# KatiaJDL/CenterPoly

Hardware: AMD Instinct MI355X
Metric: inference img/s @2048x1024 DLA-34 (1 GPU) (higher is better)
Workload: dtype f32 I/O; split-bf16 x3 contraction (a*b ~ ah*bh + ah*bl + al*bh on bf16 MFMA, ~2^-16 per product) in the convolutions, the heads and DCNv2; f32 accumulate; 1 GPU; BASELINE config 2: DLA-34 + DCNv2, 1x3x1024x2048 synthetic, 16-vertex cartesian head, K=128, forward + sigmoid + NMS/top-k/decode; parallelism=single

## Files before the change

### centerpoly_amd/_C.py

```python
import ctypes
import os
from ctypes import POINTER, Structure, c_char_p, c_float, c_int32, c_int64, c_size_t, c_void_p

import torch

_HERE = os.path.dirname(os.path.abspath(__file__))
LIB_PATH = os.path.join(_HERE, "csrc", "libcenterpoly_hip.so")

CP_OK = 0
REP = {"cartesian": 0, "polar": 1, "polar_fixed": 2}
HEATMAP_UMICH, HEATMAP_ELLIPSE = 0, 1
L1_PLAIN, L1_POLAR, L1_POLAR_FIXED, L1_RELU20, L1_SMOOTH = 0, 1, 2, 3, 4
DCN_BWD_EXACT_F32, DCN_BWD_NARROW_TILES = 1, 2
DCN_CONTRACTION = {"f32": 0, "bf16x3": 1, "bf16x3_region": 3}


class DcnShape(Structure):
    _fields_ = [(n, c_int32) for n in ("B", "Cin", "H", "W", "Cout", "kh", "kw", "stride", "pad",
                                       "dil", "deformable_groups")]


class TargetShape(Structure):
    _fields_ = [(n, c_int32) for n in ("B", "max_objs", "nbr_points", "num_classes", "out_h", "out_w",
                                       "rep", "no_reorder_flip")]
# ... 54 lines not shown
    "cp_color_aug_normalize": (c_int32, [_P, c_int64, c_int32, _P, _P, _P, _P, _P, _P, c_size_t, _P]),
    "cp_sample_inputs_workspace_bytes": (c_size_t, [c_int32] * 3),
    "cp_sample_inputs_batch": (c_int32, [_P] * 7 + [c_int32] * 3 + [_P, _P, c_size_t, _P]),
    "cp_instance_masks": (c_int32, [_P, _P, c_int32, c_int32, c_int32, c_int32, _P, _P, _P]),
    "cp_writer_instances": (c_int32, [_P, c_int32, c_int32, c_float, _P, c_int32, _P, _P, _P, _P, _P, _P, _P]),
    "cp_class_instance_masks": (c_int32, [_P, _P, _P, c_int32, c_int32, c_int32, c_int32, _P, _P, _P]),
    "cp_class_writer_instances": (c_int32, [_P, c_int32, c_int32, c_float, c_int32, _P, c_int32] + [_P] * 9),
    "cp_annot_id_instances_workspace_bytes": (c_size_t, []),
    "cp_annot_id_instances": (c_int32, [_P, c_int32, c_int32, _P, c_int32, c_int32, c_int32, _P, _P, _P, _P, _P,
                                        c_size_t, _P]),
    "cp_polygon_masks_workspace_bytes": (c_size_t, [c_int32, c_int32]),
    "cp_polygon_masks": (c_int32, [_P, _P, c_int32, c_int32, c_int32, _P, _P, _P, c_size_t, _P]),
    "cp_annot_rays_ids": (c_int32, [_P, c_int32, c_int32, _P, _P, c_int32, c_int32, _P, _P]),
    "cp_annot_rays_masks": (c_int32, [_P, c_int32, c_int32, _P, c_int32, c_int32, _P, _P]),
    "cp_polygon_paint_workspace_bytes": (c_size_t, [c_int32, c_int32]),
    "cp_polygon_paint": (c_int32, [_P, _P, _P, c_int32, c_int32, c_int32, c_int32, _P, _P, c_size_t, _P]),
    "cp_render_overlay_workspace_bytes": (c_size_t, [c_int32, c_int32]),
    "cp_render_overlay": (c_int32, [_P, c_int32, c_int32, _P, c_int32, c_int32, _P, _P, _P, _P, c_int32, _P, c_int32, _P,
                                    c_int32, _P, _P, _P, c_size_t, _P]),
    "cp_render_heatmap": (c_int32, [_P, c_int32, c_int32, c_int32, c_int32, _P, _P, _P, _P, c_int32, c_int32, _P, _P]),
    "cp_oracle_map": (c_int32, [_P, _P] + [c_int32] * 5 + [_P, _P]),
    "cp_id_histogram": (c_int32, [_P, c_int32, c_int32, _P, _P]),
    "cp_instance_overlaps_workspace_bytes": (c_size_t, [c_int32] * 4),
    "cp_instance_overlaps": (c_int32, [_P, c_int32, _P, c_int32, c_int32, _P, c_int32, _P, c_int32, _P, _P, _P, _P,
                                       c_size_t, _P]),
    "cp_polydet_post_process": (c_int32, [_P, _P, c_float, c_int32, c_int32, c_int32, _P, _P]),
    "cp_polydet_targets_workspace_bytes": (c_size_t, [POINTER(TargetShape)]),
    "cp_polydet_targets": (c_int32, [POINTER(TargetShape)] + [_P] * 19 + [_P, c_size_t, _P]),
    "cp_polydet_targets_ex": (c_int32, [POINTER(TargetShape), c_int32] + [_P] * 19 + [_P, c_size_t, _P]),
    "cp_polydet_dense_targets": (c_int32, [POINTER(TargetShape), _P, _P, c_size_t, _P, _P, _P]),
    "cp_conv_direct_supported": (c_int32, [c_int32] * 5),
    "cp_conv_direct_wgrad_supported": (c_int32, [c_int32] * 5),
    "cp_conv_direct_wgrad": (c_int32, [_P, _P, _P] + [c_int32] * 8 + [_P]),
    "cp_conv_direct_forward": (c_int32, [_P, _P, _P, _P] + [c_int32] * 9 + [_P]),
    "cp_conv_direct_forward_ex": (c_int32, [_P, _P, _P, _P] + [c_int32] * 10 + [_P]),
    "cp_conv3x3_mfma_supported": (c_int32, [c_int32] * 4),
    "cp_conv3x3_mfma_weight_bytes": (c_size_t, [c_int32] * 2),
    "cp_conv3x3_mfma_prepare": (c_int32, [_P, c_int32, c_int32, c_int32, _P, _P]),
    "cp_conv3x3_mfma_forward": (c_int32, [_P, _P, _P, _P, _P] + [c_int32] * 6 + [_P]),
    "cp_conv_mfma_weight_bytes": (c_size_t, [c_int32] * 3),
    "cp_conv_mfma_prepare": (c_int32, [_P, c_int32, c_int32, c_int32, c_int32, _P, _P]),
    "cp_conv3x3_s2_wgrad_supported": (c_int32, [c_int32] * 4),
    "cp_conv3x3_s2_wgrad": (c_int32, [_P, _P, _P] + [c_int32] * 5 + [_P]),
    "cp_conv7x7_c3_supported": (c_int32, [c_int32] * 4),
    "cp_conv7x7_c3_weight_bytes": (c_size_t, [c_int32]),
    "cp_conv7x7_c3_prepare": (c_int32, [_P, c_int32, _P, _P]),
    "cp_conv7x7_c3_forward": (c_int32, [_P, _P, _P, _P] + [c_int32] * 6 + [_P]),
    "cp_conv_mfma_prepare_blocks": (c_int32, [c_int32] * 3),
    "cp_conv_mfma_prepare_batch": (c_int32, [_P, c_int32, c_int32, _P]),
    "cp_conv_mfma_forward": (c_int32, [_P, _P, c_int32, _P, _P, _P, _P] + [c_int32] * 6 + [_P]),
    "cp_conv_mfma_forward_strided": (c_int32, [_P, _P, c_int32, _P, _P, _P, _P] + [c_int32] * 7 + [_P]),
    "cp_dla_base_pair_supported": (c_int32, [c_int32] * 2),
    "cp_dla_base_pair_forward": (c_int32, [_P] * 6 + [c_int32] * 3 + [_P]),
    "cp_conv_mfma_forward_split": (c_int32, [_P, c_int32, _P, _P, _P, _P] + [c_int32] * 9 + [_P]),
    "cp_activation_split": (c_int32, [_P, _P] + [c_int32] * 4 + [_P]),
    "cp_activation_unsplit": (c_int32, [_P, _P] + [c_int32] * 4 + [_P]),
    "cp_conv1x1_stream_supported": (c_int32, [_P, c_int32, c_int32, c_int32, c_int32]),
    "cp_conv1x1_stream_weight_bytes": (c_size_t, [c_int32] * 2),
    "cp_conv1x1_stream_prepare": (c_int32, [_P, c_int32, c_int32, _P, _P]),
    "cp_conv1x1_stream_forward": (c_int32, [_P, _P, c_int32, _P, _P, _P, _P] + [c_int32] * 5 + [_P]),
    "cp_conv1x1_stream_form": (c_int32, [c_int32] * 5),
    "cp_conv1x1_stream_forward_form": (c_int32, [_P, _P, c_int32, _P, _P, _P, _P] + [c_int32] * 7 + [_P]),
    "cp_conv3x3_stream_supported": (c_int32, [c_int32] * 4),
    "cp_conv3x3_stream_form": (c_int32, [c_int32] * 5),
    "cp_conv3x3_stream_forward": (c_int32, [_P] * 5 + [c_int32] * 6 + [_P]),
    "cp_conv3x3_stream_forward_form": (c_int32, [_P] * 5 + [c_int32] * 8 + [_P]),
    "cp_conv_mfma_input_grad_relu_workspace_bytes": (c_size_t, [c_int32] * 4),
    "cp_conv_mfma_input_grad_relu": (c_int32, [_P] * 5 + [c_int32] * 6 + [_P, c_size_t, _P]),
    "cp_conv3x3_s2_input_grad": (c_int32, [_P, _P, _P, _P] + [c_int32] * 5 + [_P]),
    "cp_conv3x3_mfma_wgrad_supported": (c_int32, [c_int32] * 4),
    "cp_conv3x3_mfma_wgrad": (c_int32, [_P, _P, _P] + [c_int32] * 5 + [_P]),
    "cp_conv_mfma_wgrad": (c_int32, [_P, _P, _P] + [c_int32] * 6 + [_P]),
    "cp_heads_fused_w2_bytes": (c_size_t, [c_int32]),
    "cp_heads_fused_prepare_w2": (c_int32, [_P, c_int32, c_int32, _P, _P]),
    "cp_heads_fused_forward": (c_int32, [_P, _P, _P, _P, _P, _P, _P] + [c_int32] * 6 + [_P]),
    "cp_maxpool2x2_forward": (c_int32, [_P, _P] + [c_int32] * 4 + [_P]),
    "cp_maxpool2x2_backward": (c_int32, [_P, _P, _P] + [c_int32] * 4 + [_P]),
    "cp_conv1x1_act_forward": (c_int32, [_P, c_int64, _P, c_int32, _P, _P, _P, c_int32, c_int32, c_int32, c_int64, _P]),
    "cp_soft_nms": (c_int32, [_P, c_int32, c_int32, c_float, c_float, c_float, c_int32]),
    "cp_soft_nms_device": (c_int32, [_P, c_int32, _P, _P, c_int32, c_float, c_float, c_float, c_int32, _P, _P]),
    "cp_merge_detections_workspace_bytes": (c_size_t, [c_int32] * 4),
    "cp_merge_detections": (c_int32, [_P] + [c_int32] * 6 + [c_float] * 3 + [c_int32, _P, _P, _P, c_size_t, _P]),
    "cp_polydet_decode_workspace_bytes": (c_size_t, [c_int32] * 5),
    "cp_polydet_decode": (c_int32, [_P, _P, _P, _P] + [c_int32] * 7 + [_P, _P, _P, _P, c_size_t, _P]),
    "cp_polydet_decode_ex": (c_int32, [_P, _P, _P, _P] + [c_int32] * 8 + [_P, _P, _P, _P, c_size_t, _P]),
    "cp_sigmoid_focal_workspace_bytes": (c_size_t, [c_int64]),
    "cp_sigmoid_focal_forward": (c_int32, [_P, _P, c_int64, _P, _P, _P, c_size_t, _P]),
    "cp_sigmoid_focal_backward": (c_int32, [_P, _P, c_int64, _P, _P, _P, _P]),
    "cp_gather_l1_forward": (c_int32, [_P, _P, _P, _P, _P] + [c_int32] * 6 + [c_float, _P, _P]),
    "cp_gather_l1_backward": (c_int32, [_P, _P, _P, _P, _P] + [c_int32] * 6 + [c_float, _P, _P, _P]),
    "cp_mse_workspace_bytes": (c_size_t, []),
    "cp_mse_forward": (c_int32, [_P, _P, c_int64, _P, _P, c_size_t, _P]),
    "cp_mse_backward": (c_int32, [_P, _P, c_int64, _P, _P, _P]),
    "cp_dense_l1_workspace_bytes": (c_size_t, []),
    "cp_dense_l1_forward": (c_int32, [_P, _P, _P, c_int64, c_float, _P, _P, c_size_t, _P]),
    "cp_dense_l1_backward": (c_int32, [_P, _P, _P, c_int64, _P, _P, _P, _P]),
    "cp_poly_iou_order_workspace_bytes": (c_size_t, [c_int32] * 3),
    "cp_poly_iou_order_forward": (c_int32, [_P, _P, _P, _P] + [c_int32] * 6 + [_P, _P, _P, _P,
                                                                               c_size_t, _P]),
    "cp_poly_iou_order_backward": (c_int32, [_P, _P, _P, _P] + [c_int32] * 6 + [_P, _P, _P, _P,
                                                                                c_size_t, _P]),
}

EXPORTS = tuple(_SIGNATURES)


# ... 52 lines not shown

    def release(self):
        self.block, self.off, self.key = None, 0, None

    def take(self, shape, device):
        n = 1
        for d in shape:
            n *= int(d)
        nbytes = (n * 4 + 255) // 256 * 256
        if nbytes > self.BLOCK // 8 or n == 0:
            return torch.zeros(tuple(shape), dtype=torch.float32, device=device)
        dev = torch.device(device)
        if dev.type == "cuda" and dev.index is None:
            dev = torch.device("cuda", torch.cuda.current_device())
        key = (dev, torch.cuda.current_stream(dev).cuda_stream)
        if self.block is None or self.key != key or self.off + nbytes > self.BLOCK:
            self.block = torch.zeros(self.BLOCK // 4, dtype=torch.float32, device=device)
            self.off, self.key = 0, key
        t = self.block[self.off // 4: self.off // 4 + n].view(tuple(shape))
        self.off += nbytes
        return t


_zero_pool = _ZeroPool()


def zeros(shape, device):
    return _zero_pool.take(shape, device)


def release_zero_pool():
    _zero_pool.release()


class _NoEvent(object):
    def record(self):
        pass


class KernelTimer(object):

    def __init__(self, watch=None):
        self.records = {}
        self.watch = watch

    def start(self, key):
        if self.watch is not None and key not in self.watch:
            return _NoEvent()
        ev = (torch.cuda.Event(enable_timing=True), torch.cuda.Event(enable_timing=True))
        self.records.setdefault(key, []).append(ev)
        ev[0].record()
        return ev[1]

    def summary(self):
        torch.cuda.synchronize()
        out = {}
        for key, evs in self.records.items():
            ms = [a.elapsed_time(b) for a, b in evs]
            out[key] = {"launches": len(ms), "avg_ms": sum(ms) / len(ms), "min_ms": min(ms)}
        return out


kernel_timer = None
```

### centerpoly_amd/models/networks/conv3x3.py

```python

import weakref

import torch
import torch.nn.functional as F

from ... import _C
from .prepared import prepared

_ENABLED = True
_WGRAD = True
MIN_CIN = 24
MIN_WORKGROUPS = 128
STREAM_1X1 = "auto"
STREAM_3X3 = "auto"


def _workgroups(B, cout, H, W):
    return B * ((W + 31) // 32) * ((H + 3) // 4) * ((cout + 31) // 32)


def _fills(B, cin, cout, H, W):
    n = _workgroups(B, cout, H, W)
    return n >= MIN_WORKGROUPS or (cin >= 256 and n >= 16)

# ... 231 lines not shown
    return out


def block_infer(x, conv1, wb1, conv2, wb2, skip):
    planes = wb1[0].shape[0]
    if not (_ENABLED and x.is_cuda and planes % 32 == 0 and tuple(wb1[0].shape[2:]) == (3, 3)
            and tuple(wb2[0].shape[2:]) == (3, 3) and conv2.stride == (1, 1)):
        return None
    B, _, H, W = x.shape
    s = conv1.stride[0]
    Ho, Wo = (H - 1) // s + 1, (W - 1) // s + 1
    if planes < MIN_CIN or not _fills(B, planes, planes, Ho, Wo) \
            or not _C.lib().cp_conv3x3_mfma_supported(planes, planes, Ho, Wo) or (skip is not None and not skip.is_contiguous()):
        return None
    y = conv_infer([x], conv1, wb1[0], wb1[1], None, True, conv=conv1, out_split=True)
    if y is None:
        return None
    z = conv_infer([y], conv2, wb2[0], wb2[1], skip, True, conv=conv2, x_split=True)
    if z is None:
        raise _C.NativeError("block_infer: the second convolution refused a split tensor its first convolution wrote")
    return z


def s2_input_grad(xshape, weight, go):
    L = _C.lib()
    B, cin, H, W = xshape
    cout = weight.shape[0]
    Ho, Wo = (H - 1) // 2 + 1, (W - 1) // 2 + 1
    if not (_ENABLED and go.is_cuda and go.dtype == torch.float32 and tuple(weight.shape[2:]) == (3, 3)
            and tuple(go.shape) == (B, cout, Ho, Wo) and cout >= MIN_CIN and L.cp_conv3x3_mfma_supported(cout, cin, Ho, Wo)
            and cin * H * W * 4 < 0x7FFFFFF0 and _fills(B, cout, cin, Ho, Wo)):
        return None
    go = go.contiguous()
    gx = torch.empty(xshape, dtype=torch.float32, device=go.device)
    end = _C.kernel_timer.start(("conv3x3s2_igrad", cout, cin, Ho, Wo, B)) if _C.kernel_timer is not None else None
    wp = _prepare(weight, cout, cin, 6)
    _C.check(L.cp_conv3x3_s2_input_grad(_C.ptr(go), _C.ptr(wp), None, _C.ptr(gx), B, cin, H, W, cout, _C.stream()),
             "cp_conv3x3_s2_input_grad")
    if end is not None:
        end.record()
    return gx


def stem_infer(x, conv, w, bias, relu):
    if not (_ENABLED and x.is_cuda and x.dtype == torch.float32 and x.dim() == 4 and conv.kernel_size == (7, 7)
            and conv.stride in ((1, 1), (2, 2)) and conv.padding == (3, 3) and conv.dilation == (1, 1) and conv.groups == 1
            and conv.in_channels == 3 and x.shape[1] == 3 and conv.padding_mode == "zeros"):
        return None
    L = _C.lib()
    B, _, H, W = x.shape
    cout, stride = w.shape[0], conv.stride[0]
    if not L.cp_conv7x7_c3_supported(cout, H, W, stride) or B > 65535:
        return None

    def build():
        wp = torch.empty(L.cp_conv7x7_c3_weight_bytes(cout), dtype=torch.uint8, device=w.device)
        _C.check(L.cp_conv7x7_c3_prepare(_C.ptr(w.contiguous()), cout, _C.ptr(wp), _C.stream()), "cp_conv7x7_c3_prepare")
        return wp
    wp, _ = prepared(conv, "stem", (w,), build)
    out = torch.empty((B, cout, (H - 1) // stride + 1, (W - 1) // stride + 1), dtype=torch.float32, device=x.device)
    _C.check(L.cp_conv7x7_c3_forward(_C.ptr(x.contiguous()), _C.ptr(wp), _C.ptr(bias), _C.ptr(out), B, H, W, cout,
                                     stride, 1 if relu else 0, _C.stream()), "cp_conv7x7_c3_forward")
    return out


def s2_weight_grad(x, weight, go):
    L = _C.lib()
    B, cin, H, W = x.shape
    cout = weight.shape[0]
    if not (_ENABLED and _WGRAD and x.is_cuda and x.dtype == torch.float32 and tuple(weight.shape[2:]) == (3, 3)
            and cin >= MIN_CIN and L.cp_conv3x3_s2_wgrad_supported(cin, cout, H, W)
            and tuple(go.shape) == (B, cout, (H - 1) // 2 + 1, W // 2)):
        return None
    gw = _C.zeros(weight.shape, weight.device)
    end = _C.kernel_timer.start(("conv3x3s2_wgrad", cin, cout, H, W, B)) if _C.kernel_timer is not None else None
    _C.check(L.cp_conv3x3_s2_wgrad(_C.ptr(x), _C.ptr(go.contiguous()), _C.ptr(gw), B, cin, H, W, cout, _C.stream()),
             "cp_conv3x3_s2_wgrad")
    if end is not None:
        end.record()
    return gw


class _Conv3x3Fn(torch.autograd.Function):

    @staticmethod
    def forward(ctx, x, weight, stride=1):
        ctx.save_for_backward(x, weight)
        ctx.stride = stride
        cout, cin = weight.shape[0], weight.shape[1]
        return _launch(x, _prepare(weight, cin, cout, False), None, None, cout, False, weight.shape[2] * weight.shape[3],
                       stride)

    @staticmethod
    def backward(ctx, go):
        x, weight = ctx.saved_tensors
        go = go.contiguous()
        if ctx.stride != 1:
            gx = None
            if ctx.needs_input_grad[0]:
                gx = s2_input_grad(x.shape, weight, go)
                if gx is None:
                    gx = torch.nn.grad.conv2d_input(x.shape, weight, go, stride=ctx.stride, padding=1)
            gw = None
            if ctx.needs_input_grad[1]:
                gw = s2_weight_grad(x, weight, go)
                if gw is None:
                    gw = torch.nn.grad.conv2d_weight(x, weight.shape, go, stride=ctx.stride, padding=1)
            return gx, gw, None
        return grads(x, weight, go, ctx.needs_input_grad[0], ctx.needs_input_grad[1], min_k=MIN_CIN) + (None,)


class _Conv3x3SkipFn(torch.autograd.Function):

    @staticmethod
    def forward(ctx, x, weight):
        ctx.save_for_backward(x, weight)
# ... 234 lines not shown
```

### centerpoly_amd/models/networks/pose_dla_dcn.py

```python
import math
import os

import numpy as np
import torch
import torch.nn.functional as F
from torch import nn

from ... import _C
from .DCNv2.dcn_v2 import DCN, conv_bias
from . import conv3x3
from .conv3x3 import conv_infer, conv_raw
from .prepared import prepared, release_inference

HEADS_FUSED = True
CONV_DIRECT_WGRAD = True

BN_MOMENTUM = 0.1


def _bn(c):
    return nn.BatchNorm2d(c, momentum=BN_MOMENTUM)



# ... 57 lines not shown
        gx = gw = None
        if weight.shape[2] == 3 and stride == 1 and pad == 1 and conv3x3.mfma_enabled():
            gx, gw = conv3x3.grads(x, weight, go, ctx.needs_input_grad[0], ctx.needs_input_grad[1] and not direct_w)
        elif ctx.needs_input_grad[0]:
            if weight.shape[2] == 3 and stride == 2 and pad == 1 and conv3x3.mfma_enabled():
                gx = conv3x3.s2_input_grad(tuple(x.shape), weight, go)
            if gx is None:
                gx = torch.nn.grad.conv2d_input(x.shape, weight, go, stride=stride, padding=pad)
        if ctx.needs_input_grad[1] and gw is None:
            L = _C.lib()
            B, cin, H, W = x.shape
            cout, k = weight.shape[0], weight.shape[2]
            if direct_w and L.cp_conv_direct_wgrad_supported(cin, cout, k, stride, pad):
                gw = _C.zeros(weight.shape, weight.device)
                rc = L.cp_conv_direct_wgrad(_C.ptr(x), _C.ptr(go), _C.ptr(gw), B, cin, H, W, cout, k, stride, pad,
                                            _C.stream())
                if rc == -2:
                    gw = None
                else:
                    _C.check(rc, "cp_conv_direct_wgrad")
            if gw is None:
                gw = torch.nn.grad.conv2d_weight(x, weight.shape, go, stride=stride, padding=pad)
        return gx, gw, None, None


def conv_train(conv, x):
    kh, kw = conv.kernel_size
    if (x.is_cuda and x.dtype == torch.float32 and conv.bias is None and kh == kw and conv.groups == 1
            and conv.dilation == (1, 1) and conv.stride[0] == conv.stride[1] and conv.padding[0] == conv.padding[1]
            and x.shape[1] * x.shape[2] * x.shape[3] * 4 < 0x70000000
            and _C.lib().cp_conv_direct_supported(conv.in_channels, conv.out_channels, kh, conv.stride[0],
                                                  conv.padding[0])):
        return _DirectConvFn.apply(x.contiguous(), conv.weight, conv.stride[0], conv.padding[0])
    if conv.bias is None:
        return conv_raw(conv, x)
    return conv(x)


def _base_pair(dla, x):
    c0, c1 = dla.level0[0], dla.level1[0]
    if not (x.is_cuda and x.dtype == torch.float32 and x.dim() == 4 and conv3x3.mfma_enabled()
            and (c0.in_channels, c0.out_channels, c0.kernel_size, c0.stride, c0.padding, c0.dilation, c0.groups)
            == (16, 16, (3, 3), (1, 1), (1, 1), (1, 1), 1)
            and (c1.in_channels, c1.out_channels, c1.kernel_size, c1.stride, c1.padding, c1.dilation, c1.groups)
            == (16, 32, (3, 3), (2, 2), (1, 1), (1, 1), 1)):
        return None
    B, _, H, W = x.shape
    L = _C.lib()
    if not L.cp_dla_base_pair_supported(H, W) or B > 65535:
        return None
    (w0, b0), (w1, b1) = dla._folded[1], dla._folded[2]
    x = x.contiguous()
    out = torch.empty((B, 32, (H - 1) // 2 + 1, (W - 1) // 2 + 1), dtype=torch.float32, device=x.device)
    end = _C.kernel_timer.start(("conv_base_pair", 16, 32, H, W, B)) if _C.kernel_timer is not None else None
    rc = L.cp_dla_base_pair_forward(_C.ptr(x), _C.ptr(w0.contiguous()), _C.ptr(b0), _C.ptr(w1.contiguous()), _C.ptr(b1),
                                    _C.ptr(out), B, H, W, _C.stream())
    if rc == -2:
        return None
    _C.check(rc, "cp_dla_base_pair_forward")
    if end is not None:
        end.record()
    return out


def _conv_folded(x, conv, wb, relu=False, residual=None):
    if residual is None:
        y = None
        if conv.kernel_size == (7, 7) and x.is_cuda:
            y = conv3x3.stem_infer(x, conv, wb[0], wb[1], relu)
        if y is None:
            y = _conv_direct(x, conv, wb, relu)
        if y is not None:
            return y
    if x.is_cuda:
        y = conv_infer([x], conv, wb[0], wb[1], residual, relu, conv=conv)
        if y is not None:
            return y
    if not x.is_cuda:
        y = F.conv2d(x, wb[0], wb[1], conv.stride, conv.padding, conv.dilation, conv.groups)
        if residual is not None:
            y = y + residual
        return F.relu_(y) if relu else y
    y = F.conv2d(x, wb[0], None, conv.stride, conv.padding, conv.dilation, conv.groups)
    B, C, H, W = y.shape
    if not y.is_contiguous() or (H * W) % 4 != 0 or (residual is not None and not residual.is_contiguous()):
        y = y + wb[1].view(1, -1, 1, 1)
        if residual is not None:
            y = y + residual
        return F.relu_(y) if relu else y
    rc = _C.lib().cp_bias_act_inplace(_C.ptr(y), _C.ptr(wb[1]), _C.ptr(residual), B, C, H * W,
                                      1 if relu else 0, _C.stream())
    _C.check(rc, "cp_bias_act_inplace")
    return y


class _MaxPool2x2Fn(torch.autograd.Function):

    @staticmethod
    def forward(ctx, x):
        B, C, H, W = x.shape
        out = torch.empty((B, C, H // 2, W // 2), dtype=torch.float32, device=x.device)
        _C.check(_C.lib().cp_maxpool2x2_forward(_C.ptr(x), _C.ptr(out), B, C, H, W, _C.stream()), "cp_maxpool2x2_forward")
        ctx.save_for_backward(x)
        return out

    @staticmethod
    def backward(ctx, go):
        (x,) = ctx.saved_tensors
        B, C, H, W = x.shape
        gx = torch.empty_like(x)
        _C.check(_C.lib().cp_maxpool2x2_backward(_C.ptr(x), _C.ptr(go.contiguous()), _C.ptr(gx), B, C, H, W,
                                                 _C.stream()), "cp_maxpool2x2_backward")
# ... 222 lines not shown
                    if bottom.is_cuda:
                        bn_act(self.project[1], conv_train(self.project[0], bottom), relu=False)
                    else:
                        self.project(bottom)
        elif _use_folded(self):
            residual = _conv_folded(bottom, self.project[0], self._folded)
        else:
            residual = bn_act(self.project[1], conv_train(self.project[0], bottom), relu=False)
        if self.level_root:
            children.append(bottom)
        if Tree.share_pool and self.levels > 1 and not torch.is_grad_enabled() and self._same_pool(self.tree1):
            x1 = self.tree1(x, residual, bottom=bottom)
        else:
            x1 = self.tree1(x, residual)
        if self.levels == 1:
            return self.root(self.tree2(x1), x1, *children)
        children.append(x1)
        return self.tree2(x1, children=children)


class DLA(nn.Module):
    def __init__(self, levels, channels, num_classes=1000, block=BasicBlock, residual_root=False,
                 linear_root=False):
        super().__init__()
        self.channels, self.num_classes = channels, num_classes
        c = channels
        self.base_layer = nn.Sequential(nn.Conv2d(3, c[0], 7, 1, 3, bias=False), _bn(c[0]),
                                        nn.ReLU(inplace=True))
        self.level0 = self._conv_level(c[0], c[0], levels[0])
        self.level1 = self._conv_level(c[0], c[1], levels[1], stride=2)
        for i in range(2, 6):
            setattr(self, "level%d" % i, Tree(levels[i], block, c[i - 1], c[i], 2,
                                              level_root=i > 2, root_residual=residual_root))

    @staticmethod
    def _conv_level(inplanes, planes, convs, stride=1, dilation=1):
        mods = []
        for i in range(convs):
            mods += [nn.Conv2d(inplanes, planes, 3, stride if i == 0 else 1, dilation, dilation,
                               bias=False), _bn(planes), nn.ReLU(inplace=True)]
            inplanes = planes
        return nn.Sequential(*mods)

    def fold(self):
        seqs = (self.base_layer, self.level0, self.level1)
        if any(len(seq) != 3 for seq in seqs):
            self._folded = None
            return
        self._folded = [_fold_conv_bn(seq[0], seq[1]) for seq in seqs]

    def forward(self, x):
        pyramid = []
        if _use_folded(self):
            x = _conv_folded(x, self.base_layer[0], self._folded[0], relu=True)
            y1 = _base_pair(self, x) if getattr(self, "skip_level0_output", False) else None
            if y1 is not None:
                pyramid += [None, y1]
                x = y1
            else:
                for seq, wb in zip((self.level0, self.level1), self._folded[1:]):
                    x = _conv_folded(x, seq[0], wb, relu=True)
                    pyramid.append(x)
            first_tree = 2
        elif self.training and x.is_cuda and all(len(q) == 3 for q in (self.base_layer, self.level0,
                                                                        self.level1)):
            for seq in (self.base_layer, self.level0, self.level1):
                x = bn_act(seq[1], conv_train(seq[0], x), relu=True)
                if seq is not self.base_layer:
                    pyramid.append(x)
            first_tree = 2
        else:
            x = self.base_layer(x)
            first_tree = 0
        for i in range(first_tree, 6):
            x = getattr(self, "level%d" % i)(x)
            pyramid.append(x)
        return pyramid

    def load_pretrained_model(self, data="imagenet", name="dla34", hash="ba72cf86"):
        if not name.endswith(".pth"):
            raise RuntimeError("no network: pass a local ImageNet checkpoint as name='*.pth'")
        weights = torch.load(data + name, map_location="cpu")
        self.load_state_dict(weights, strict=False)


def dla34(pretrained=False, **kwargs):
    model = DLA([1, 1, 1, 2, 2, 1], [16, 32, 64, 128, 256, 512], block=BasicBlock, **kwargs)
    if pretrained:
        model.load_pretrained_model(data="imagenet", name="dla34", hash="ba72cf86")
    return model


def fill_up_weights(up):
    w = up.weight.data
    k = w.size(2)
    f = math.ceil(k / 2)
    c = (2 * f - 1 - f % 2) / (2.0 * f)
    tri = torch.tensor([1 - abs(i / f - c) for i in range(k)], dtype=w.dtype)
    w[:, 0] = torch.outer(tri, tri[:w.size(3)])


def fill_fc_weights(layers):
    for m in layers.modules():
        if isinstance(m, nn.Conv2d) and m.bias is not None:
            nn.init.constant_(m.bias, 0)


class DeformConv(nn.Module):
# ... 322 lines not shown
```

### include/centerpoly_hip.h

```cpp
#ifndef CENTERPOLY_HIP_H
#define CENTERPOLY_HIP_H

#include <stddef.h>
#include <stdint.h>

#ifdef __cplusplus
extern "C" {
#endif

#define CP_ABI_VERSION 3

enum {
  CP_OK = 0,
  CP_EINVAL = -1,
  CP_EUNSUPPORTED = -2,
  CP_EWORKSPACE = -3,
  CP_EHIP = -4
};

enum { CP_REP_CARTESIAN = 0, CP_REP_POLAR = 1, CP_REP_POLAR_FIXED = 2 };

enum {
  CP_DCN_F32 = 0,
  CP_DCN_BF16X3 = 1,
// ... 62 lines not shown
                                   const float* ep_shift, int32_t relu, const float* weight, const float* skip,
                                   float* out, int32_t B, int32_t C, int32_t H, int32_t W, int32_t f, void* stream);
int cp_depthwise_up_backward(const float* x, const float* weight, const float* grad_out,
                             float* grad_x, float* grad_weight, int32_t B, int32_t C, int32_t H,
                             int32_t W, int32_t f, void* stream);

int cp_maxpool2x2_forward(const float* x, float* out, int32_t B, int32_t C, int32_t H, int32_t W, void* stream);
int cp_maxpool2x2_backward(const float* x, const float* grad_out, float* grad_in, int32_t B, int32_t C, int32_t H,
                           int32_t W, void* stream);

int cp_upsample2x_add(const float* a, const float* low, float* out, int32_t B, int32_t C, int32_t H, int32_t W,
                      void* stream);

int cp_bias_act_inplace(float* y, const float* bias, const float* residual, int32_t B, int32_t C,
                        int64_t HW, int32_t relu, void* stream);
int cp_bias_relu_backward(const float* y, const float* grad_out, float* grad_in, float* grad_bias,
                          int32_t B, int32_t C, int64_t HW, void* stream);
int cp_channel_sum_accumulate(const float* x, float* out, int32_t B, int32_t C, int64_t HW, void* stream);

int cp_conv_direct_supported(int32_t Cin, int32_t Cout, int32_t k, int32_t stride, int32_t pad);
int cp_conv_direct_forward(const float* x, const float* w, const float* bias, float* out, int32_t B, int32_t Cin,
                           int32_t H, int32_t W, int32_t Cout, int32_t k, int32_t stride, int32_t pad,
                           int32_t relu, void* stream);
int cp_conv_direct_forward_ex(const float* x, const float* w, const float* bias, float* out, int32_t B, int32_t Cin,
                           int32_t H, int32_t W, int32_t Cout, int32_t k, int32_t stride, int32_t pad,
                           int32_t relu, int32_t split_bf16, void* stream);

int cp_conv3x3_mfma_supported(int32_t Cin, int32_t Cout, int32_t H, int32_t W);
size_t cp_conv3x3_mfma_weight_bytes(int32_t Cin, int32_t Cout);
int cp_conv3x3_mfma_prepare(const float* weight, int32_t Cin, int32_t Cout, int32_t transposed, void* wperm,
                            void* stream);
int cp_conv3x3_mfma_forward(const float* x, const void* wperm, const float* bias, const float* residual, float* out,
                            int32_t B, int32_t Cin, int32_t H, int32_t W, int32_t Cout, int32_t relu, void* stream);

size_t cp_conv_mfma_weight_bytes(int32_t Cin, int32_t Cout, int32_t taps);
int cp_conv_mfma_prepare(const float* weight, int32_t Cin, int32_t Cout, int32_t taps, int32_t transposed, void* wperm,
                         void* stream);
typedef struct cp_conv_prepare_job {
  const float* weight;
  void* wperm;
  int32_t Cin, Cout, taps, transposed, first_block, reserved;
} cp_conv_prepare_job;
int32_t cp_conv_mfma_prepare_blocks(int32_t Cin, int32_t Cout, int32_t taps);
int cp_conv_mfma_prepare_batch(const cp_conv_prepare_job* jobs_device, int32_t njobs, int32_t total_blocks, void* stream);
int cp_conv_mfma_forward(const float* const* xs, const int32_t* cs, int32_t nsrc, const void* wperm, const float* bias,
                         const float* residual, float* out, int32_t B, int32_t H, int32_t W, int32_t Cout,
                         int32_t taps, int32_t relu, void* stream);
int cp_conv_mfma_forward_strided(const float* const* xs, const int32_t* cs, int32_t nsrc, const void* wperm,
                                 const float* bias, const float* residual, float* out, int32_t B, int32_t H, int32_t W,
                                 int32_t Cout, int32_t taps, int32_t stride, int32_t relu, void* stream);
int cp_dla_base_pair_supported(int32_t H, int32_t W);
int cp_dla_base_pair_forward(const float* x, const float* w0, const float* b0, const float* w1, const float* b1, float* out,
                             int32_t B, int32_t H, int32_t W, void* stream);
int cp_conv_mfma_forward_split(const void* x, int32_t x_split, const void* wperm, const float* bias, const float* residual,
                               void* out, int32_t out_split, int32_t B, int32_t Cin, int32_t H, int32_t W, int32_t Cout,
                               int32_t taps, int32_t stride, int32_t relu, void* stream);
int cp_activation_split(const float* x, void* out, int32_t B, int32_t C, int32_t H, int32_t W, void* stream);
int cp_activation_unsplit(const void* in, float* x, int32_t B, int32_t C, int32_t H, int32_t W, void* stream);
int cp_conv1x1_stream_supported(const int32_t* cs, int32_t nsrc, int32_t Cout, int32_t H, int32_t W);
size_t cp_conv1x1_stream_weight_bytes(int32_t Cin, int32_t Cout);
int cp_conv1x1_stream_prepare(const float* weight, int32_t Cin, int32_t Cout, void* wperm, void* stream);
int cp_conv1x1_stream_forward(const float* const* xs, const int32_t* cs, int32_t nsrc, const void* wperm, const float* bias,
                              const float* residual, float* out, int32_t B, int32_t H, int32_t W, int32_t Cout,
                              int32_t relu, void* stream);
int cp_conv1x1_stream_form(int32_t Cin, int32_t Cout, int32_t H, int32_t W, int32_t B);
int cp_conv1x1_stream_forward_form(const float* const* xs, const int32_t* cs, int32_t nsrc, const void* wperm,
                                   const float* bias, const float* residual, float* out, int32_t B, int32_t H, int32_t W,
                                   int32_t Cout, int32_t relu, int32_t nb, int32_t ks, void* stream);
int cp_conv3x3_stream_supported(int32_t Cin, int32_t Cout, int32_t H, int32_t W);
int cp_conv3x3_stream_form(int32_t Cin, int32_t Cout, int32_t H, int32_t W, int32_t B);
int cp_conv3x3_stream_forward(const float* x, const void* wperm, const float* bias, const float* residual, float* out,
                              int32_t B, int32_t Cin, int32_t H, int32_t W, int32_t Cout, int32_t relu, void* stream);
int cp_conv3x3_stream_forward_form(const float* x, const void* wperm, const float* bias, const float* residual, float* out,
                                   int32_t B, int32_t Cin, int32_t H, int32_t W, int32_t Cout, int32_t relu, int32_t nt,
                                   int32_t ks, void* stream);
int cp_conv3x3_s2_wgrad_supported(int32_t Cin, int32_t Cout, int32_t H, int32_t W);
int cp_conv3x3_s2_wgrad(const float* x, const float* grad_out, float* gw, int32_t B, int32_t Cin, int32_t H, int32_t W,
                        int32_t Cout, void* stream);

int cp_conv7x7_c3_supported(int32_t Cout, int32_t H, int32_t W, int32_t stride);
size_t cp_conv7x7_c3_weight_bytes(int32_t Cout);
int cp_conv7x7_c3_prepare(const float* weight, int32_t Cout, void* wperm, void* stream);
int cp_conv7x7_c3_forward(const float* x, const void* wperm, const float* bias, float* out, int32_t B, int32_t H,
                          int32_t W, int32_t Cout, int32_t stride, int32_t relu, void* stream);

size_t cp_conv_mfma_input_grad_relu_workspace_bytes(int32_t B, int32_t Cin, int32_t H, int32_t W);
int cp_conv_mfma_input_grad_relu(const float* grad_out, const void* wperm_t, const float* y, float* grad_y,
                                 float* grad_bias, int32_t B, int32_t Cin, int32_t H, int32_t W, int32_t Cout,
                                 int32_t taps, void* workspace, size_t workspace_bytes, void* stream);
int cp_conv3x3_s2_input_grad(const float* grad_out, const void* wperm_t, const float* residual, float* grad_in, int32_t B,
                             int32_t Cin, int32_t H, int32_t W, int32_t Cout, void* stream);

int cp_conv3x3_mfma_wgrad_supported(int32_t Cin, int32_t Cout, int32_t H, int32_t W);
int cp_conv3x3_mfma_wgrad(const float* x, const float* go, float* gw, int32_t B, int32_t Cin, int32_t H, int32_t W,
                          int32_t Cout, void* stream);
int cp_conv_mfma_wgrad(const float* x, const float* go, float* gw, int32_t B, int32_t Cin, int32_t H, int32_t W,
                       int32_t Cout, int32_t taps, void* stream);

int cp_conv_direct_wgrad_supported(int32_t Cin, int32_t Cout, int32_t k, int32_t stride, int32_t pad);
int cp_conv_direct_wgrad(const float* x, const float* go, float* gw, int32_t B, int32_t Cin, int32_t H, int32_t W,
                         int32_t Cout, int32_t k, int32_t stride, int32_t pad, void* stream);

size_t cp_heads_fused_w2_bytes(int32_t head_conv);
int cp_heads_fused_prepare_w2(const float* w2, int32_t cout, int32_t head_conv, void* w2perm, void* stream);
int cp_heads_fused_forward(const float* x, const void* wperm1, const float* b1, const void* const* w2perm,
                           const float* const* b2, float* const* out, const int32_t* cout, int32_t nheads, int32_t B,
// ... 191 lines not shown
```

Measured before the change: 391.5 img/s.

## Fuse DLA stem 7x7 conv with level0/level1 convs into one persistent kernel

```diff
diff --git a/centerpoly_amd/_C.py b/centerpoly_amd/_C.py
--- a/centerpoly_amd/_C.py
+++ b/centerpoly_amd/_C.py
@@ -130,6 +130,8 @@
     "cp_conv_mfma_forward_strided": (c_int32, [_P, _P, c_int32, _P, _P, _P, _P] + [c_int32] * 7 + [_P]),
     "cp_dla_base_pair_supported": (c_int32, [c_int32] * 2),
     "cp_dla_base_pair_forward": (c_int32, [_P] * 6 + [c_int32] * 3 + [_P]),
+    "cp_dla_base_trio_supported": (c_int32, [c_int32] * 2),
+    "cp_dla_base_trio_forward": (c_int32, [_P] * 8 + [c_int32] * 3 + [_P]),
     "cp_conv_mfma_forward_split": (c_int32, [_P, c_int32, _P, _P, _P, _P] + [c_int32] * 9 + [_P]),
     "cp_activation_split": (c_int32, [_P, _P] + [c_int32] * 4 + [_P]),
     "cp_activation_unsplit": (c_int32, [_P, _P] + [c_int32] * 4 + [_P]),
@@ -288,6 +290,13 @@
         ev[0].record()
         return ev[1]
 
+    def drop(self, key, end):
+        evs = self.records.get(key)
+        if evs and evs[-1][1] is end:
+            evs.pop()
+            if not evs:
+                del self.records[key]
+
     def summary(self):
         torch.cuda.synchronize()
         out = {}
diff --git a/centerpoly_amd/csrc/conv_base_trio.hip b/centerpoly_amd/csrc/conv_base_trio.hip
--- /dev/null
+++ b/centerpoly_amd/csrc/conv_base_trio.hip
@@ -0,0 +1,396 @@
+#include <type_traits>
+
+#include "cp_common.h"
+
+namespace {
+
+typedef __bf16 tbf16x8 __attribute__((ext_vector_type(8)));
+typedef __bf16 tbf16x2 __attribute__((ext_vector_type(2)));
+typedef float tf32x2 __attribute__((ext_vector_type(2)));
+typedef unsigned tu32x4 __attribute__((ext_vector_type(4)));
+typedef unsigned tu32x2 __attribute__((ext_vector_type(2)));
+
+constexpr unsigned TOOB = 0x80000000u;
+constexpr int NT = 512, NWG = 256;
+constexpr int CIN = 16, C1 = 32, KS = 5;
+constexpr int SKS = 6, SPAIRS = 21;
+constexpr int TW2 = 32;
+constexpr int L0W = 2 * TW2 + 1, LR = 8;
+constexpr int XW = 72, XR = 8;
+constexpr int RR = 12, RP = XW + 5;
+constexpr int NSEG = XW / 4;
+constexpr int XHALF = XR * XW * 16, L0HALF = LR * L0W * 16, RPLANE = 3 * RR * RP * 16;
+constexpr int LDS_BYTES = 2 * RPLANE + 4 * XHALF + 4 * L0HALF;
+static_assert(3 * 4 * NSEG <= NT, "one staging item per thread");
+static_assert(C1 * CIN * 9 * 4 <= 2 * RPLANE, "the raw weights fit the region they pass through");
+static_assert(LDS_BYTES <= 160 * 1024, "one workgroup per CU");
+
+struct TrioArgs {
+  const float* image;
+  const tbf16x8* wp;
+  const float* bs;
+  const float* w0;
+  const float* b0;
+  const float* w1;
+  const float* b1;
+  float* out;
+  int H, W, Ho, Wo;
+  int strips, run_rows, items_per_image, nitems;
+};
+
+__device__ __forceinline__ void tsplit2(float v0, float v1, unsigned& hi, unsigned& lo) {
+  const tbf16x2 h = __builtin_convertvector(tf32x2{v0, v1}, tbf16x2);
+  const unsigned hb = __builtin_bit_cast(unsigned, h);
+  const float h0 = __builtin_bit_cast(float, hb << 16), h1 = __builtin_bit_cast(float, hb & 0xffff0000u);
+  const tbf16x2 l = __builtin_convertvector(tf32x2{v0 - h0, v1 - h1}, tbf16x2);
+  hi = hb;
+  lo = __builtin_bit_cast(unsigned, l);
+}
+
+__device__ __forceinline__ int rslot(int cell) { return cell + ((cell + 14) >> 4); }
+
+__global__ __launch_bounds__(NT, 1) void conv_base_trio_kernel(TrioArgs a) {
+  __shared__ __attribute__((aligned(16))) unsigned char rec[2 * RPLANE];
+  __shared__ __attribute__((aligned(16))) unsigned char xs[4 * XHALF];
+  __shared__ __attribute__((aligned(16))) unsigned char ls[4 * L0HALF];
+
+  const int tid = threadIdx.x, lane = tid & 63;
+  const int wid = __builtin_amdgcn_readfirstlane(tid >> 6);
+  const int lpx = lane & 15, g = lane >> 4;
+  const int HW = a.H * a.W;
+  const int cm = wid & 1;
+
+  tbf16x8 sa[SKS][2], wh0[KS], wl0[KS], wh1[KS], wl1[KS];
+#pragma unroll
+  for (int s_ = 0; s_ < SKS; ++s_) {
+    sa[s_][0] = a.wp[(s_ * 2 + 0) * 64 + lane];
+    sa[s_][1] = a.wp[(s_ * 2 + 1) * 64 + lane];
+  }
+  {
+    float* wsh = reinterpret_cast<float*>(rec);
+    for (int i = tid; i < CIN * CIN * 9; i += NT) wsh[i] = a.w0[i];
+    __syncthreads();
+#pragma unroll
+    for (int s_ = 0; s_ < KS; ++s_) {
+      const int tap = 2 * s_ + (g >> 1);
+#pragma unroll
+      for (int j = 0; j < 8; ++j) {
+        const float w = tap < 9 ? wsh[(lpx * CIN + 8 * (g & 1) + j) * 9 + tap] : 0.f;
+        const __bf16 h = (__bf16)w;
+        wh0[s_][j] = h;
+        wl0[s_][j] = (__bf16)(w - (float)h);
+      }
+    }
+    __syncthreads();
+    for (int i = tid; i < C1 * CIN * 9; i += NT) wsh[i] = a.w1[i];
+    __syncthreads();
+#pragma unroll
+    for (int s_ = 0; s_ < KS; ++s_) {
+      const int tap = 2 * s_ + (g >> 1);
+#pragma unroll
+      for (int j = 0; j < 8; ++j) {
+        const float w = tap < 9 ? wsh[((16 * cm + lpx) * CIN + 8 * (g & 1) + j) * 9 + tap] : 0.f;
+        const __bf16 h = (__bf16)w;
+        wh1[s_][j] = h;
+        wl1[s_][j] = (__bf16)(w - (float)h);
+      }
+    }
+    __syncthreads();
+  }
+  float bsr[4], b0r[4], b1r[4];
+#pragma unroll
+  for (int q = 0; q < 4; ++q) {
+    bsr[q] = a.bs ? a.bs[4 * g + q] : 0.f;
+    b0r[q] = a.b0 ? a.b0[4 * g + q] : 0.f;
+    b1r[q] = a.b1 ? a.b1[16 * cm + 4 * g + q] : 0.f;
+  }
+  int sky[SKS], sci[SKS];
+#pragma unroll
+  for (int s_ = 0; s_ < SKS; ++s_) {
+    const int pair = min(4 * s_ + g, SPAIRS - 1);
+    sky[s_] = pair / 3;
+    sci[s_] = (pair - 3 * sky[s_]) * (RR * RP * 16);
+  }
+  int tky[KS], tkx[KS];
+#pragma unroll
+  for (int s_ = 0; s_ < KS; ++s_) {
+    const int tap = min(2 * s_ + (g >> 1), 8);
+    tky[s_] = tap / 3;
+    tkx[s_] = tap - 3 * tky[s_];
+  }
+
+  const int itid = tid - NT / 2;
+  const bool item = itid >= 0 && itid < 3 * 4 * NSEG;
+  const int ici = max(itid, 0) / (4 * NSEG), irow = (max(itid, 0) / NSEG) & 3, iseg = max(itid, 0) % NSEG;
+  f32x4 v[3];
+
+  struct Step {
+    int it, k, b, x0, Y0, ns;
+  };
+  auto decode = [&](Step& s) {
+    s.b = s.it / a.items_per_image;
+    const int r = s.it - s.b * a.items_per_image;
+    const int run = r / a.strips;
+    s.x0 = (r - run * a.strips) * TW2;
+    s.Y0 = run * a.run_rows;
+    s.ns = (min(a.run_rows, a.Ho - s.Y0) + 1) >> 1;
+  };
+  auto next_step = [&](const Step& s) {
+    Step n = s;
+    if (s.it >= a.nitems) return n;
+    n.k = s.k + 1;
+    if (n.k >= s.ns) {
+      n.it = s.it + gridDim.x;
+      n.k = -3;
+      if (n.it < a.nitems) decode(n);
+    }
+    return n;
+  };
+  auto km12 = [](int k) { return (4 * k + 24) % 12; };
+  auto km8 = [](int k) { return (4 * k + 16) & 7; };
+
+  auto load_item = [&](const Step& s) {
+    const int gy = 2 * s.Y0 + 4 * s.k + 4 + irow, gx0 = 2 * s.x0 - 8 + 4 * iseg;
+    const bool rok = item && s.it < a.nitems && gy >= 0 && gy < a.H;
+    const __amdgpu_buffer_rsrc_t rs = __builtin_amdgcn_make_buffer_rsrc(
+        const_cast<float*>(a.image + (long long)(s.it < a.nitems ? s.b : 0) * 3 * HW), 0, (int)(3u * (unsigned)HW * 4u),
+        0x00020000);
+#pragma unroll
+    for (int j = 0; j < 3; ++j) {
+      const int gx = gx0 + 4 * j;
+      const unsigned off = (rok && gx >= 0 && gx < a.W) ? ((unsigned)ici * (unsigned)HW + (unsigned)(gy * a.W + gx)) * 4u : TOOB;
+      v[j] = __builtin_bit_cast(f32x4, __builtin_amdgcn_raw_buffer_load_b128(rs, off, 0, 0));
+    }
+  };
+  auto write_records = [&](const Step& s) {
+    if (!item) return;
+    unsigned ph[6], pl[6];
+#pragma unroll
+    for (int j = 0; j < 3; ++j) {
+      tsplit2(v[j][0], v[j][1], ph[2 * j], pl[2 * j]);
+      tsplit2(v[j][2], v[j][3], ph[2 * j + 1], pl[2 * j + 1]);
+    }
+    int rr = km12(s.k) + 4 + irow;
+    rr = rr >= RR ? rr - RR : rr;
+    unsigned char* rowp = rec + ((ici * RR + rr) * RP) * 16;
+#pragma unroll
+    for (int r = 0; r < 4; ++r) {
+      tu32x4 rh, rl;
+      if ((r & 1) == 0) {
+        const int p = r / 2;
+        rh = tu32x4{ph[p], ph[p + 1], ph[p + 2], ph[p + 3]};
+        rl = tu32x4{pl[p], pl[p + 1], pl[p + 2], pl[p + 3]};
+      } else {
+        const int p = (r - 1) / 2;
+#pragma unroll
+        for (int j = 0; j < 4; ++j) {
+          rh[j] = __builtin_amdgcn_alignbit(ph[p + j + 1], ph[p + j], 16);
+          rl[j] = __builtin_amdgcn_alignbit(pl[p + j + 1], pl[p + j], 16);
+        }
+      }
+      unsigned char* dst = rowp + rslot(4 * iseg + r) * 16;
+      *reinterpret_cast<tu32x4*>(dst) = rh;
+      *reinterpret_cast<tu32x4*>(dst + RPLANE) = rl;
+    }
+  };
+
+  auto stage_a = [&](const Step& s, auto nc) {
+    constexpr int NCH = decltype(nc)::value;
+    const int k12 = km12(s.k), k8 = km8(s.k);
+    int crow[NCH], ccell[NCH];
+    bool cval[NCH];
+#pragma unroll
+    for (int n = 0; n < NCH; ++n) {
+      if (n < 2) {
+        crow[n] = (wid >> 2) + 2 * n;
+        ccell[n] = 2 + 16 * (wid & 3) + lpx;
+        cval[n] = true;
+      } else {
+        const int r = lpx / 3;
+        crow[n] = min(r, 3);
+        cval[n] = lpx < 12;
+        ccell[n] = cval[n] ? 66 + (lpx - 3 * r) : 66;
+      }
+    }
+    f32x4 acc[NCH];
+#pragma unroll
+    for (int n = 0; n < NCH; ++n) acc[n] = f32x4{0.f, 0.f, 0.f, 0.f};
+#pragma unroll
+    for (int s_ = 0; s_ < SKS; ++s_) {
+      tbf16x8 bh[NCH], bl[NCH];
+#pragma unroll
+      for (int n = 0; n < NCH; ++n) {
+        int t = k12 + 10 + crow[n] + sky[s_];
+        t = t >= 2 * RR ? t - 2 * RR : (t >= RR ? t - RR : t);
+        const unsigned char* p = rec + sci[s_] + (t * RP + rslot(ccell[n])) * 16;
+        bh[n] = *reinterpret_cast<const tbf16x8*>(p);
+        bl[n] = *reinterpret_cast<const tbf16x8*>(p + RPLANE);
+      }
+#pragma unroll
+      for (int n = 0; n < NCH; ++n) acc[n] = __builtin_amdgcn_mfma_f32_16x16x32_bf16(sa[s_][0], bh[n], acc[n], 0, 0, 0);
+#pragma unroll
+      for (int n = 0; n < NCH; ++n) acc[n] = __builtin_amdgcn_mfma_f32_16x16x32_bf16(sa[s_][0], bl[n], acc[n], 0, 0, 0);
+#pragma unroll
+      for (int n = 0; n < NCH; ++n) acc[n] = __builtin_amdgcn_mfma_f32_16x16x32_bf16(sa[s_][1], bh[n], acc[n], 0, 0, 0);
+    }
+#pragma unroll
+    for (int n = 0; n < NCH; ++n) {
+      if (!cval[n]) continue;
+      const int sy = 2 * s.Y0 + 4 * s.k + 1 + crow[n], sx = 2 * s.x0 - 4 + ccell[n];
+      const bool inside = sy >= 0 && sy < a.H && sx >= 0 && sx < a.W;
+      float o[4];
+#pragma unroll
+      for (int q = 0; q < 4; ++q) o[q] = inside ? fmaxf(acc[n][q] + bsr[q], 0.f) : 0.f;
+      unsigned hi[2], lo[2];
+      tsplit2(o[0], o[1], hi[0], lo[0]);
+      tsplit2(o[2], o[3], hi[1], lo[1]);
+      const int rr = (k8 + 1 + crow[n]) & 7;
+      unsigned char* dst = xs + (g >> 1) * XHALF + (rr * XW + ccell[n]) * 16 + (g & 1) * 8;
+      *reinterpret_cast<tu32x2*>(dst) = tu32x2{hi[0], hi[1]};
+      *reinterpret_cast<tu32x2*>(dst + 2 * XHALF) = tu32x2{lo[0], lo[1]};
+    }
+  };
+
+  auto stage_b = [&](const Step& s, auto nc) {
+    constexpr int NCH = decltype(nc)::value;
+    const int k8 = km8(s.k);
+    int crow[NCH], ccol[NCH];
+    bool cval[NCH];
+#pragma unroll
+    for (int n = 0; n < NCH; ++n) {
+      if (n < 2) {
+        crow[n] = (wid >> 2) + 2 * n;
+        ccol[n] = 16 * (wid & 3) + lpx;
+        cval[n] = true;
+      } else {
+        crow[n] = min(lpx, 3);
+        ccol[n] = L0W - 1;
+        cval[n] = lpx < 4;
+      }
+    }
+    f32x4 acc[NCH];
+#pragma unroll
+    for (int n = 0; n < NCH; ++n) acc[n] = f32x4{0.f, 0.f, 0.f, 0.f};
+#pragma unroll
+    for (int s_ = 0; s_ < KS; ++s_) {
+      tbf16x8 bh[NCH], bl[NCH];
+#pragma unroll
+      for (int n = 0; n < NCH; ++n) {
+        const int rr = (k8 + 7 + crow[n] + tky[s_]) & 7;
+        const unsigned char* p = xs + (g & 1) * XHALF + (rr * XW + ccol[n] + 2 + tkx[s_]) * 16;
+        bh[n] = *reinterpret_cast<const tbf16x8*>(p);
+        bl[n] = *reinterpret_cast<const tbf16x8*>(p + 2 * XHALF);
+      }
+#pragma unroll
+      for (int n = 0; n < NCH; ++n) acc[n] = __builtin_amdgcn_mfma_f32_16x16x32_bf16(wh0[s_], bh[n], acc[n], 0, 0, 0);
+#pragma unroll
+      for (int n = 0; n < NCH; ++n) acc[n] = __builtin_amdgcn_mfma_f32_16x16x32_bf16(wh0[s_], bl[n], acc[n], 0, 0, 0);
+#pragma unroll
+      for (int n = 0; n < NCH; ++n) acc[n] = __builtin_amdgcn_mfma_f32_16x16x32_bf16(wl0[s_], bh[n], acc[n], 0, 0, 0);
+    }
+#pragma unroll
+    for (int n = 0; n < NCH; ++n) {
+      if (!cval[n]) continue;
+      const int iy = 2 * s.Y0 + 4 * s.k + crow[n], ix = 2 * s.x0 - 1 + ccol[n];
+      const bool inside = iy >= 0 && iy < a.H && ix >= 0 && ix < a.W;
+      float o[4];
+#pragma unroll
+      for (int q = 0; q < 4; ++q) o[q] = inside ? fmaxf(acc[n][q] + b0r[q], 0.f) : 0.f;
+      unsigned hi[2], lo[2];
+      tsplit2(o[0], o[1], hi[0], lo[0]);
+      tsplit2(o[2], o[3], hi[1], lo[1]);
+      const int rr = (k8 + crow[n]) & 7;
+      unsigned char* dst = ls + (g >> 1) * L0HALF + (rr * L0W + ccol[n]) * 16 + (g & 1) * 8;
+      *reinterpret_cast<tu32x2*>(dst) = tu32x2{hi[0], hi[1]};
+      *reinterpret_cast<tu32x2*>(dst + 2 * L0HALF) = tu32x2{lo[0], lo[1]};
+    }
+  };
+
+  auto stage_c = [&](const Step& s) {
+    const int k8 = km8(s.k);
+    const int row = wid >> 2, x2 = ((wid >> 1) & 1) * 16 + lpx;
+    f32x4 acc = f32x4{0.f, 0.f, 0.f, 0.f};
+#pragma unroll
+    for (int s_ = 0; s_ < KS; ++s_) {
+      const int rr = (k8 + 7 + 2 * row + tky[s_]) & 7;
+      const unsigned char* p = ls + (g & 1) * L0HALF + (rr * L0W + 2 * x2 + tkx[s_]) * 16;
+      const tbf16x8 bh = *reinterpret_cast<const tbf16x8*>(p);
+      const tbf16x8 bl = *reinterpret_cast<const tbf16x8*>(p + 2 * L0HALF);
+      acc = __builtin_amdgcn_mfma_f32_16x16x32_bf16(wh1[s_], bh, acc, 0, 0, 0);
+      acc = __builtin_amdgcn_mfma_f32_16x16x32_bf16(wh1[s_], bl, acc, 0, 0, 0);
+      acc = __builtin_amdgcn_mfma_f32_16x16x32_bf16(wl1[s_], bh, acc, 0, 0, 0);
+    }
+    const int oy = s.Y0 + 2 * s.k + row, ox = s.x0 + x2;
+    if (oy < a.Ho && ox < a.Wo) {
+      float* ob = a.out + (long long)s.b * C1 * a.Ho * a.Wo;
+#pragma unroll
+      for (int q = 0; q < 4; ++q)
+        ob[((long long)(16 * cm + 4 * g + q) * a.Ho + oy) * a.Wo + ox] = fmaxf(acc[q] + b1r[q], 0.f);
+    }
+  };
+
+  Step prv, cur, nxt;
+  cur.it = blockIdx.x;
+  cur.k = -3;
+  cur.b = cur.x0 = cur.Y0 = cur.ns = 0;
+  decode(cur);
+  prv = cur;
+  load_item(cur);
+  write_records(cur);
+  nxt = next_step(cur);
+  load_item(nxt);
+  __syncthreads();
+#pragma unroll 1
+  while (cur.it < a.nitems) {
+    if (cur.k >= -1) {
+      if (wid == 7) stage_a(cur, std::integral_constant<int, 3>());
+      else stage_a(cur, std::integral_constant<int, 2>());
+    }
+    if (prv.k >= 0) stage_c(prv);
+    __syncthreads();
+    if (cur.k >= -1) {
+      if (wid == 0) stage_b(cur, std::integral_constant<int, 3>());
+      else stage_b(cur, std::integral_constant<int, 2>());
+    }
+    if (nxt.it < a.nitems) write_records(nxt);
+    const Step n2 = next_step(nxt);
+    load_item(n2);
+    __syncthreads();
+    prv = cur;
+    cur = nxt;
+    nxt = n2;
+  }
+  if (prv.k >= 0) stage_c(prv);
+}
+
+}
+
+extern "C" int cp_dla_base_trio_supported(int32_t H, int32_t W) {
+  return H >= 1 && W >= 4 && (W & 3) == 0 && (unsigned long long)CIN * H * W * 4ull < 0x70000000ull;
+}
+
+extern "C" int cp_dla_base_trio_forward(const float* image, const void* stem_wperm, const float* stem_bias, const float* w0,
+                                        const float* b0, const float* w1, const float* b1, float* out, int32_t B, int32_t H,
+                                        int32_t W, void* stream) {
+  CP_CHECK_ARG(image && stem_wperm && w0 && w1 && out && B >= 1 && B <= 65535);
+  if (!cp_dla_base_trio_supported(H, W) || (reinterpret_cast<unsigned long long>(image) & 15)) return CP_EUNSUPPORTED;
+  TrioArgs a;
+  a.image = image; a.wp = (const tbf16x8*)stem_wperm; a.bs = stem_bias;
+  a.w0 = w0; a.b0 = b0; a.w1 = w1; a.b1 = b1; a.out = out;
+  a.H = H; a.W = W; a.Ho = (H - 1) / 2 + 1; a.Wo = (W - 1) / 2 + 1;
+  a.strips = (a.Wo + TW2 - 1) / TW2;
+  const long long columns = (long long)a.strips * B;
+  long long nruns = (NWG + columns - 1) / columns;
+  const long long cap = (a.Ho + 31) / 32;
+  nruns = nruns < cap ? nruns : cap;
+  int rows = (int)((a.Ho + nruns - 1) / nruns);
+  rows += rows & 1;
+  a.run_rows = rows;
+  a.items_per_image = a.strips * ((a.Ho + rows - 1) / rows);
+  const long long nitems = (long long)a.items_per_image * B;
+  if (nitems > 0x3FFFFFFFll) return CP_EUNSUPPORTED;
+  a.nitems = (int)nitems;
+  const int wgs = (int)(nitems < NWG ? nitems : NWG);
+  hipLaunchKernelGGL(conv_base_trio_kernel, dim3(wgs), dim3(NT), 0, (hipStream_t)stream, a);
+  return cp_launch_status();
+}
diff --git a/centerpoly_amd/models/networks/conv3x3.py b/centerpoly_amd/models/networks/conv3x3.py
--- a/centerpoly_amd/models/networks/conv3x3.py
+++ b/centerpoly_amd/models/networks/conv3x3.py
@@ -307,16 +307,22 @@
     cout, stride = w.shape[0], conv.stride[0]
     if not L.cp_conv7x7_c3_supported(cout, H, W, stride) or B > 65535:
         return None
+    wp = stem_prepared(conv, w)
+    out = torch.empty((B, cout, (H - 1) // stride + 1, (W - 1) // stride + 1), dtype=torch.float32, device=x.device)
+    _C.check(L.cp_conv7x7_c3_forward(_C.ptr(x.contiguous()), _C.ptr(wp), _C.ptr(bias), _C.ptr(out), B, H, W, cout,
+                                     stride, 1 if relu else 0, _C.stream()), "cp_conv7x7_c3_forward")
+    return out
+
+
+def stem_prepared(conv, w):
+    L = _C.lib()
+    cout = w.shape[0]
 
     def build():
         wp = torch.empty(L.cp_conv7x7_c3_weight_bytes(cout), dtype=torch.uint8, device=w.device)
         _C.check(L.cp_conv7x7_c3_prepare(_C.ptr(w.contiguous()), cout, _C.ptr(wp), _C.stream()), "cp_conv7x7_c3_prepare")
         return wp
-    wp, _ = prepared(conv, "stem", (w,), build)
-    out = torch.empty((B, cout, (H - 1) // stride + 1, (W - 1) // stride + 1), dtype=torch.float32, device=x.device)
-    _C.check(L.cp_conv7x7_c3_forward(_C.ptr(x.contiguous()), _C.ptr(wp), _C.ptr(bias), _C.ptr(out), B, H, W, cout,
-                                     stride, 1 if relu else 0, _C.stream()), "cp_conv7x7_c3_forward")
-    return out
+    return prepared(conv, "stem", (w,), build)[0]
 
 
 def s2_weight_grad(x, weight, go):
diff --git a/centerpoly_amd/models/networks/pose_dla_dcn.py b/centerpoly_amd/models/networks/pose_dla_dcn.py
--- a/centerpoly_amd/models/networks/pose_dla_dcn.py
+++ b/centerpoly_amd/models/networks/pose_dla_dcn.py
@@ -133,12 +133,51 @@
     (w0, b0), (w1, b1) = dla._folded[1], dla._folded[2]
     x = x.contiguous()
     out = torch.empty((B, 32, (H - 1) // 2 + 1, (W - 1) // 2 + 1), dtype=torch.float32, device=x.device)
-    end = _C.kernel_timer.start(("conv_base_pair", 16, 32, H, W, B)) if _C.kernel_timer is not None else None
+    key = ("conv_base_pair", 16, 32, H, W, B)
+    end = _C.kernel_timer.start(key) if _C.kernel_timer is not None else None
     rc = L.cp_dla_base_pair_forward(_C.ptr(x), _C.ptr(w0.contiguous()), _C.ptr(b0), _C.ptr(w1.contiguous()), _C.ptr(b1),
                                     _C.ptr(out), B, H, W, _C.stream())
     if rc == -2:
+        if end is not None:
+            _C.kernel_timer.drop(key, end)
         return None
     _C.check(rc, "cp_dla_base_pair_forward")
+    if end is not None:
+        end.record()
+    return out
+
+
+BASE_TRIO = "auto"
+
+
+def _base_trio(dla, x):
+    cs, c0, c1 = dla.base_layer[0], dla.level0[0], dla.level1[0]
+    if not (BASE_TRIO != "off" and x.is_cuda and x.dtype == torch.float32 and x.dim() == 4 and x.shape[1] == 3
+            and conv3x3.mfma_enabled()
+            and (cs.in_channels, cs.out_channels, cs.kernel_size, cs.stride, cs.padding, cs.dilation, cs.groups,
+                 cs.padding_mode) == (3, 16, (7, 7), (1, 1), (3, 3), (1, 1), 1, "zeros")
+            and (c0.in_channels, c0.out_channels, c0.kernel_size, c0.stride, c0.padding, c0.dilation, c0.groups)
+            == (16, 16, (3, 3), (1, 1), (1, 1), (1, 1), 1)
+            and (c1.in_channels, c1.out_channels, c1.kernel_size, c1.stride, c1.padding, c1.dilation, c1.groups)
+            == (16, 32, (3, 3), (2, 2), (1, 1), (1, 1), 1)):
+        return None
+    B, _, H, W = x.shape
+    L = _C.lib()
+    if not L.cp_dla_base_trio_supported(H, W) or B > 65535:
+        return None
+    (ws, bs), (w0, b0), (w1, b1) = dla._folded
+    wp = conv3x3.stem_prepared(cs, ws)
+    x = x.contiguous()
+    out = torch.empty((B, 32, (H - 1) // 2 + 1, (W - 1) // 2 + 1), dtype=torch.float32, device=x.device)
+    key = ("conv_base_trio", 3, 32, H, W, B)
+    end = _C.kernel_timer.start(key) if _C.kernel_timer is not None else None
+    rc = L.cp_dla_base_trio_forward(_C.ptr(x), _C.ptr(wp), _C.ptr(bs), _C.ptr(w0.contiguous()), _C.ptr(b0),
+                                    _C.ptr(w1.contiguous()), _C.ptr(b1), _C.ptr(out), B, H, W, _C.stream())
+    if rc == -2:
+        if end is not None:
+            _C.kernel_timer.drop(key, end)
+        return None
+    _C.check(rc, "cp_dla_base_trio_forward")
     if end is not None:
         end.record()
     return out
@@ -467,8 +506,11 @@
     def forward(self, x):
         pyramid = []
         if _use_folded(self):
-            x = _conv_folded(x, self.base_layer[0], self._folded[0], relu=True)
-            y1 = _base_pair(self, x) if getattr(self, "skip_level0_output", False) else None
+            skip0 = getattr(self, "skip_level0_output", False)
+            y1 = _base_trio(self, x) if skip0 else None
+            if y1 is None:
+                x = _conv_folded(x, self.base_layer[0], self._folded[0], relu=True)
+                y1 = _base_pair(self, x) if skip0 else None
             if y1 is not None:
                 pyramid += [None, y1]
                 x = y1
diff --git a/include/centerpoly_hip.h b/include/centerpoly_hip.h
--- a/include/centerpoly_hip.h
+++ b/include/centerpoly_hip.h
@@ -138,6 +138,10 @@
 int cp_dla_base_pair_supported(int32_t H, int32_t W);
 int cp_dla_base_pair_forward(const float* x, const float* w0, const float* b0, const float* w1, const float* b1, float* out,
                              int32_t B, int32_t H, int32_t W, void* stream);
+int cp_dla_base_trio_supported(int32_t H, int32_t W);
+int cp_dla_base_trio_forward(const float* image, const void* stem_wperm, const float* stem_bias, const float* w0,
+                             const float* b0, const float* w1, const float* b1, float* out, int32_t B, int32_t H,
+                             int32_t W, void* stream);
 int cp_conv_mfma_forward_split(const void* x, int32_t x_split, const void* wperm, const float* bias, const float* residual,
                                void* out, int32_t out_split, int32_t B, int32_t Cin, int32_t H, int32_t W, int32_t Cout,
                                int32_t taps, int32_t stride, int32_t relu, void* stream);
```

Result: faster. 399.2 img/s (median of 6 runs) (+2.0%).
